# Lzcstan/DrugLAMP

Hardware: AMD Instinct MI355X
Metric: drug-protein pairs/sec training step (higher is better)
Workload: dtype bf16; 1 GPU; DrugLAMP training step (cls step, epoch 1; fwd+bwd+grad all-reduce+AdamW), BindingDB-shaped synthetic pairs (512 drug nodes/tokens, 2304 protein tokens = 256 sites, pre-extracted 384-d/640-d LLM embeddings), global batch 256 = 256 per GPU x 1; per_gpu_batch=256, global_batch=256, parallelism=dp1, step_kind=cls, epoch=1, hip_graph=False, protein_seq_len=2304, distinct_batches=8, first_touch_steps=8, padding_rows=computed once, protein_cnn_rows=distinct rows, streams=independent branches on side HIP streams

## Files before the change

### druglamp_amd/csrc/attention.hip

```cpp
#include "tiles.cuh"

namespace {
using namespace dltile;

struct AttnP {
  const char *Q, *K, *V, *O, *dO;
  char *Out, *dQ, *dK, *dV;
  float *LSE, *Delta, *raw;
  int64_t q_ps, q_hs, q_rs, k_ps, k_hs, k_rs, v_ps, v_hs, v_rs, o_ps, o_hs, o_rs, o_ss;
  int64_t do_ps, do_hs, do_rs, do_ss, dq_ps, dq_hs, dq_rs, dk_ps, dk_hs, dk_rs, dv_ps, dv_hs, dv_rs;
  int P, H, S, shift, Lq, Lk;
  float scale;
  int algo;
  int tail_start;
  float tail_bias;
};

template <int QT, int NKT>
__device__ __forceinline__ void add_tail_bias_t(f32x4 (&s)[QT][NKT], int k0, int g, int tail_start, float tb) {
#pragma unroll
  for (int kt = 0; kt < NKT; ++kt)
#pragma unroll
    for (int r = 0; r < 4; ++r)
      if (k0 + kt * 16 + 4 * g + r >= tail_start) {
// ... 334 lines not shown
  const T* d = reinterpret_cast<const T*>(p.dO) + (int64_t)seg * p.do_ss + (int64_t)pr * p.do_ps +
               (int64_t)h * p.do_hs + (int64_t)q * p.do_rs;
  float s = 0.f;
#pragma unroll
  for (int c = sub * 4; c < HD; c += 64) {
    const f32x4 a = load4<T>(o + c), b = load4<T>(d + c);
    s += a[0] * b[0] + a[1] * b[1] + a[2] * b[2] + a[3] * b[3];
  }
  s += __shfl_xor(s, 8, 64); s += __shfl_xor(s, 4, 64); s += __shfl_xor(s, 2, 64); s += __shfl_xor(s, 1, 64);
  if (sub == 0) p.Delta[row] = s;
}

template <typename T, int HD, int QT, bool RES>
__global__ __launch_bounds__(ATT_THREADS, (HD == 64 ? 2 : 1)) void attn_bwd_dq_kernel(const AttnP p) {
  using TL = ATile<T, HD>;
  constexpr int KF = Mma<T>::KF, NKF = HD / KF, NDT = HD / 16, CT = KF / 16;
  constexpr int KVB = 64, NKT = KVB / 16, NKP = KVB / KF;
  constexpr int QB = 4 * QT * 16;
  constexpr int LROWS = RES ? 256 : KVB;
  __shared__ __attribute__((aligned(16))) char smem[2 * LROWS * TL::RB];
  char* Ks = smem;
  char* Vs = smem + LROWS * TL::RB;
  const int lane = threadIdx.x & 63, wave = threadIdx.x >> 6, il = lane & 15, g = lane >> 4;
  const int qb = blockIdx.x, h = blockIdx.y, pq = blockIdx.z;
  const T* Qb = reinterpret_cast<const T*>(p.Q) + (int64_t)pq * p.q_ps + (int64_t)h * p.q_hs;
  const int qw0 = qb * QB + wave * QT * 16;
  const float c = p.scale * LOG2E;

  u32x4 qf[QT][NKF];
#pragma unroll
  for (int qt = 0; qt < QT; ++qt) {
    const int q = qw0 + qt * 16 + il;
#pragma unroll
    for (int kf = 0; kf < NKF; ++kf) qf[qt][kf] = frag_global<T>(Qb + (int64_t)q * p.q_rs, q < p.Lq, kf, g);
  }
  f32x4 dq[NDT][QT];
#pragma unroll
  for (int d = 0; d < NDT; ++d)
#pragma unroll
    for (int qt = 0; qt < QT; ++qt) dq[d][qt] = f32x4{0.f, 0.f, 0.f, 0.f};

  for (int seg = 0; seg < p.S; ++seg) {
    const int pa = seg == 0 ? pq : (pq + p.P - p.shift) % p.P;
    const T* Kb = reinterpret_cast<const T*>(p.K) + (int64_t)pa * p.k_ps + (int64_t)h * p.k_hs;
    const T* Vb = reinterpret_cast<const T*>(p.V) + (int64_t)pa * p.v_ps + (int64_t)h * p.v_hs;
    const T* dOb = reinterpret_cast<const T*>(p.dO) + (int64_t)seg * p.do_ss + (int64_t)pa * p.do_ps +
                   (int64_t)h * p.do_hs;
    const int64_t statbase = (((int64_t)seg * p.P + pa) * p.H + h) * p.Lq;
    const int nt = (p.Lk + KVB - 1) / KVB;
    if constexpr (RES) {
      dma_rows<T, HD, ATT_THREADS>(Ks, Kb, p.k_rs, p.Lk, nt * KVB);
      dma_rows<T, HD, ATT_THREADS>(Vs, Vb, p.v_rs, p.Lk, nt * KVB);
    }
    u32x4 dof[QT][NKF];
    float lse2[QT], delta[QT];
#pragma unroll
    for (int qt = 0; qt < QT; ++qt) {
      const int q = qw0 + qt * 16 + il;
      const bool ok = q < p.Lq;
#pragma unroll
      for (int kf = 0; kf < NKF; ++kf) dof[qt][kf] = frag_global<T>(dOb + (int64_t)q * p.do_rs, ok, kf, g);
      lse2[qt] = ok ? p.LSE[statbase + q] * LOG2E : INFINITY;
      if constexpr (sizeof(T) == 2) {
        const T* Ob = reinterpret_cast<const T*>(p.O) + (int64_t)seg * p.o_ss + (int64_t)pa * p.o_ps + (int64_t)h * p.o_hs;
        float part = 0.f;
#pragma unroll
        for (int kf = 0; kf < NKF; ++kf) part += dot8_bf16(dof[qt][kf], frag_global<T>(Ob + (int64_t)q * p.o_rs, ok, kf, g));
        delta[qt] = group4_sum(part);
        if (ok && g == 0) p.Delta[statbase + q] = delta[qt];
      } else {
        delta[qt] = ok ? p.Delta[statbase + q] : 0.f;
      }
    }
    Stager<T, HD, KVB> sk, sv;
    if constexpr (RES) {
      __syncthreads();
    } else {
      sk.load(Kb, p.k_rs, 0, p.Lk);
      sv.load(Vb, p.v_rs, 0, p.Lk);
    }
    for (int t = 0; t < nt; ++t) {
      const int k0 = t * KVB;
      if constexpr (!RES) {
        sk.store(Ks);
        sv.store(Vs);
        __syncthreads();
        if (t + 1 < nt) {
          sk.load(Kb, p.k_rs, k0 + KVB, p.Lk);
          sv.load(Vb, p.v_rs, k0 + KVB, p.Lk);
        }
      }
      const char* Kt = RES ? Ks + k0 * TL::RB : Ks;
      const char* Vt = RES ? Vs + k0 * TL::RB : Vs;
      f32x4 s[QT][NKT], dp[QT][NKT];
#pragma unroll
      for (int kt = 0; kt < NKT; ++kt) {
#pragma unroll
        for (int qt = 0; qt < QT; ++qt) { s[qt][kt] = f32x4{0.f, 0.f, 0.f, 0.f}; dp[qt][kt] = f32x4{0.f, 0.f, 0.f, 0.f}; }
#pragma unroll
        for (int kf = 0; kf < NKF; ++kf) {
          const u32x4 ka = frag_kc<T, HD>(Kt, kt * 16, kf, il, g);
          const u32x4 va = frag_kc<T, HD>(Vt, kt * 16, kf, il, g);
#pragma unroll
          for (int qt = 0; qt < QT; ++qt) {
            s[qt][kt] = Mma<T>::mma(ka, qf[qt][kf], s[qt][kt]);
            dp[qt][kt] = Mma<T>::mma(va, dof[qt][kf], dp[qt][kt]);
          }
        }
      }
      if constexpr (!RES) { if (k0 + KVB > p.tail_start) add_tail_bias_t<QT, NKT>(s, k0, g, p.tail_start, p.tail_bias); }
#pragma unroll
      for (int qt = 0; qt < QT; ++qt)
#pragma unroll
        for (int kt = 0; kt < NKT; ++kt)
#pragma unroll
          for (int r = 0; r < 4; ++r) {
            const float pv = fast_exp2(s[qt][kt][r] * c - lse2[qt]);
            s[qt][kt][r] = pv * (dp[qt][kt][r] - delta[qt]);
          }
#pragma unroll
      for (int kp = 0; kp < NKP; ++kp) {
        u32x4 db[QT];
#pragma unroll
        for (int qt = 0; qt < QT; ++qt) db[qt] = frag_from_acc<T>(&s[qt][kp * CT]);
#pragma unroll
        for (int d = 0; d < NDT; ++d) {
          const u32x4 kta = frag_tr<T, HD>(Kt, kp * KF, d * 16, il, g);
#pragma unroll
          for (int qt = 0; qt < QT; ++qt) dq[d][qt] = Mma<T>::mma(kta, db[qt], dq[d][qt]);
        }
      }
      if constexpr (!RES) __syncthreads();
    }
    if constexpr (RES) { if (seg + 1 < p.S) __syncthreads(); }
  }
  T* dQb = reinterpret_cast<T*>(p.dQ) + (int64_t)pq * p.dq_ps + (int64_t)h * p.dq_hs;
#pragma unroll
  for (int qt = 0; qt < QT; ++qt) {
    const int q = qw0 + qt * 16 + il;
    if (q < p.Lq) {
#pragma unroll
      for (int d = 0; d < NDT; ++d)
        store4_fam<4, T>(dQb + (int64_t)q * p.dq_rs + d * 16 + 4 * g, dq[d][qt] * p.scale);
    }
  }
}

__device__ __forceinline__ void att_dma16(const char* gsrc, uint32_t lds_off) {
  asm volatile("s_mov_b32 m0, %1\n\ts_nop 0\n\tglobal_load_lds_dwordx4 %0, off" ::"v"(gsrc), "s"(lds_off) : "memory");
}
__device__ __forceinline__ void att_wait_all() { asm volatile("s_waitcnt vmcnt(0) lgkmcnt(0)" ::: "memory"); }
__device__ __forceinline__ void att_barrier() { asm volatile("s_barrier" ::: "memory"); }

template <typename T, int HD, int QT, bool TAILK = false>
__global__ __launch_bounds__(ATT_THREADS, 2) void attn_bwd_dq_ring_kernel(const AttnP p) {
  using TL = ATile<T, HD>;
  constexpr int KF = Mma<T>::KF, NKF = HD / KF, NDT = HD / 16, CT = KF / 16;
  constexpr int KVB = 64, NKP = KVB / KF;
  constexpr int QB = 4 * QT * 16;
  constexpr int TILE = KVB * TL::RB, STAGE = 2 * TILE;
  constexpr int NCH = KVB * TL::CPR / ATT_THREADS;
  static_assert(sizeof(T) == 2 && KVB * TL::CPR % ATT_THREADS == 0, "bf16 tiles, whole DMA instructions");
  __shared__ __attribute__((aligned(16))) char smem[2 * STAGE];
  const uint32_t smem_lds = (uint32_t)(size_t)(__attribute__((address_space(3))) char*)smem;
  const int tid = threadIdx.x, lane = tid & 63, wave = tid >> 6, il = lane & 15, g = lane >> 4;
  const int qb = blockIdx.x, h = blockIdx.y, pq = blockIdx.z;
  const T* Qb = reinterpret_cast<const T*>(p.Q) + (int64_t)pq * p.q_ps + (int64_t)h * p.q_hs;
  const int qw0 = qb * QB + wave * QT * 16;
  const float c = p.scale * LOG2E;

  u32x4 qf[QT][NKF];
#pragma unroll
  for (int qt = 0; qt < QT; ++qt) {
    const int q = qw0 + qt * 16 + il;
#pragma unroll
    for (int kf = 0; kf < NKF; ++kf) qf[qt][kf] = frag_global<T>(Qb + (int64_t)q * p.q_rs, q < p.Lq, kf, g);
  }
  f32x4 dq[NDT][QT];
#pragma unroll
  for (int d = 0; d < NDT; ++d)
#pragma unroll
    for (int qt = 0; qt < QT; ++qt) dq[d][qt] = f32x4{0.f, 0.f, 0.f, 0.f};

  for (int seg = 0; seg < p.S; ++seg) {
    const int pa = seg == 0 ? pq : (pq + p.P - p.shift) % p.P;
    const T* Kb = reinterpret_cast<const T*>(p.K) + (int64_t)pa * p.k_ps + (int64_t)h * p.k_hs;
    const T* Vb = reinterpret_cast<const T*>(p.V) + (int64_t)pa * p.v_ps + (int64_t)h * p.v_hs;
    const T* dOb = reinterpret_cast<const T*>(p.dO) + (int64_t)seg * p.do_ss + (int64_t)pa * p.do_ps + (int64_t)h * p.do_hs;
    const int64_t statbase = (((int64_t)seg * p.P + pa) * p.H + h) * p.Lq;
    const int nt = (p.Lk + KVB - 1) / KVB;
    auto issue = [&](int t, int buf) {
      const char* zero = reinterpret_cast<const char*>(zero_page);
      const uint32_t sb = smem_lds + (uint32_t)buf * STAGE;
#pragma unroll
      for (int i = 0; i < NCH; ++i) {
        const int cc = tid + i * ATT_THREADS;
        const int row = cc / TL::CPR, ch = (cc % TL::CPR) ^ TL::swz(row);
        const int key = t * KVB + row;
        const char* ks = key < p.Lk ? reinterpret_cast<const char*>(Kb + (int64_t)key * p.k_rs + ch * TL::EPC) : zero;
        const char* vs = key < p.Lk ? reinterpret_cast<const char*>(Vb + (int64_t)key * p.v_rs + ch * TL::EPC) : zero;
        const uint32_t off = __builtin_amdgcn_readfirstlane((uint32_t)((wave * 64 + i * ATT_THREADS) * 16));
        att_dma16(ks, sb + off);
        att_dma16(vs, sb + TILE + off);
      }
    };
    if (seg > 0) att_barrier();
    issue(0, 0);
    u32x4 dof[QT][NKF];
    float lse2[QT], delta[QT];
#pragma unroll
    for (int qt = 0; qt < QT; ++qt) {
      const int q = qw0 + qt * 16 + il;
      const bool ok = q < p.Lq;
#pragma unroll
      for (int kf = 0; kf < NKF; ++kf) dof[qt][kf] = frag_global<T>(dOb + (int64_t)q * p.do_rs, ok, kf, g);
      lse2[qt] = ok ? p.LSE[statbase + q] * LOG2E : INFINITY;
      const T* Ob = reinterpret_cast<const T*>(p.O) + (int64_t)seg * p.o_ss + (int64_t)pa * p.o_ps + (int64_t)h * p.o_hs;
      float part = 0.f;
#pragma unroll
      for (int kf = 0; kf < NKF; ++kf) part += dot8_bf16(dof[qt][kf], frag_global<T>(Ob + (int64_t)q * p.o_rs, ok, kf, g));
      delta[qt] = group4_sum(part);
      if (ok && g == 0) p.Delta[statbase + q] = delta[qt];
    }
    for (int t = 0; t < nt; ++t) {
      att_wait_all();
      att_barrier();
      if (t + 1 < nt) issue(t + 1, (t + 1) & 1);
      const char* Kt = smem + (t & 1) * STAGE;
      const char* Vt = Kt + TILE;
#pragma unroll
      for (int kp = 0; kp < NKP; ++kp) {
        f32x4 s[QT][CT], dp[QT][CT];
#pragma unroll
        for (int ci = 0; ci < CT; ++ci) {
          const int kt = kp * CT + ci;
#pragma unroll
          for (int qt = 0; qt < QT; ++qt) { s[qt][ci] = f32x4{0.f, 0.f, 0.f, 0.f}; dp[qt][ci] = f32x4{0.f, 0.f, 0.f, 0.f}; }
#pragma unroll
          for (int kf = 0; kf < NKF; ++kf) {
            const u32x4 ka = frag_kc<T, HD>(Kt, kt * 16, kf, il, g);
            const u32x4 va = frag_kc<T, HD>(Vt, kt * 16, kf, il, g);
#pragma unroll
            for (int qt = 0; qt < QT; ++qt) {
              s[qt][ci] = Mma<T>::mma(ka, qf[qt][kf], s[qt][ci]);
              dp[qt][ci] = Mma<T>::mma(va, dof[qt][kf], dp[qt][ci]);
            }
          }
        }
        if constexpr (TAILK) {
          if (t * KVB + (kp + 1) * KF > p.tail_start) add_tail_bias_t<QT, CT>(s, t * KVB + kp * KF, g, p.tail_start, p.tail_bias);
        }
#pragma unroll
        for (int qt = 0; qt < QT; ++qt)
#pragma unroll
          for (int ci = 0; ci < CT; ++ci)
#pragma unroll
            for (int r = 0; r < 4; ++r) {
              const float pv = fast_exp2(s[qt][ci][r] * c - lse2[qt]);
              s[qt][ci][r] = pv * (dp[qt][ci][r] - delta[qt]);
            }
        u32x4 db[QT];
#pragma unroll
        for (int qt = 0; qt < QT; ++qt) db[qt] = frag_from_acc<T>(&s[qt][0]);
#pragma unroll
        for (int d = 0; d < NDT; ++d) {
          const u32x4 kta = frag_tr<T, HD>(Kt, kp * KF, d * 16, il, g);
#pragma unroll
          for (int qt = 0; qt < QT; ++qt) dq[d][qt] = Mma<T>::mma(kta, db[qt], dq[d][qt]);
        }
      }
    }
  }
  T* dQb = reinterpret_cast<T*>(p.dQ) + (int64_t)pq * p.dq_ps + (int64_t)h * p.dq_hs;
#pragma unroll
  for (int qt = 0; qt < QT; ++qt) {
    const int q = qw0 + qt * 16 + il;
    if (q < p.Lq) {
#pragma unroll
      for (int d = 0; d < NDT; ++d)
        store4_fam<4, T>(dQb + (int64_t)q * p.dq_rs + d * 16 + 4 * g, dq[d][qt] * p.scale);
    }
  }
}

template <typename T, int HD, int KT, bool RES>
__global__ __launch_bounds__(ATT_THREADS, (HD == 64 ? 2 : 1)) void attn_bwd_dkv_kernel(const AttnP p) {
  using TL = ATile<T, HD>;
  constexpr int KF = Mma<T>::KF, NKF = HD / KF, NDT = HD / 16, CT = KF / 16;
  constexpr int QSB = 64;
  constexpr int NQT = QSB / 16;
  constexpr int NQP = QSB / KF;
  constexpr int KVB = 4 * KT * 16;
  constexpr int LROWS = RES ? 256 : QSB;
  __shared__ __attribute__((aligned(16))) char smem[2 * LROWS * TL::RB + 2 * LROWS * sizeof(float)];
  char* Qs = smem;
  char* dOs = smem + LROWS * TL::RB;
  float* lse_s = reinterpret_cast<float*>(smem + 2 * LROWS * TL::RB);
  float* del_s = lse_s + LROWS;
  const int lane = threadIdx.x & 63, wave = threadIdx.x >> 6, il = lane & 15, g = lane >> 4;
  const int kb = blockIdx.x, h = blockIdx.y, pa = blockIdx.z;
  const T* Kb = reinterpret_cast<const T*>(p.K) + (int64_t)pa * p.k_ps + (int64_t)h * p.k_hs;
  const T* Vb = reinterpret_cast<const T*>(p.V) + (int64_t)pa * p.v_ps + (int64_t)h * p.v_hs;
  const int kw0 = kb * KVB + wave * KT * 16;
  const float c = p.scale * LOG2E;

  u32x4 kfr[KT][NKF], vfr[KT][NKF];
#pragma unroll
  for (int kt = 0; kt < KT; ++kt) {
    const int key = kw0 + kt * 16 + il;
    const bool ok = key < p.Lk;
#pragma unroll
    for (int kf = 0; kf < NKF; ++kf) {
      kfr[kt][kf] = frag_global<T>(Kb + (int64_t)key * p.k_rs, ok, kf, g);
      vfr[kt][kf] = frag_global<T>(Vb + (int64_t)key * p.v_rs, ok, kf, g);
    }
  }
  f32x4 dk[NDT][KT], dv[NDT][KT];
#pragma unroll
  for (int d = 0; d < NDT; ++d)
#pragma unroll
    for (int kt = 0; kt < KT; ++kt) { dk[d][kt] = f32x4{0.f, 0.f, 0.f, 0.f}; dv[d][kt] = f32x4{0.f, 0.f, 0.f, 0.f}; }
  const bool has_tail = !RES && kw0 + KT * 16 > p.tail_start;
  float kbl[KT];
#pragma unroll
  for (int kt = 0; kt < KT; ++kt) kbl[kt] = (kw0 + kt * 16 + il >= p.tail_start) ? p.tail_bias : 0.f;

  Stager<T, HD, QSB> sq, sdo;
  const int nqb = (p.Lq + QSB - 1) / QSB;
  for (int seg = 0; seg < p.S; ++seg) {
    const int qprob = seg == 0 ? pa : (pa + p.shift) % p.P;
    const T* Qb = reinterpret_cast<const T*>(p.Q) + (int64_t)qprob * p.q_ps + (int64_t)h * p.q_hs;
    const T* dOb = reinterpret_cast<const T*>(p.dO) + (int64_t)seg * p.do_ss + (int64_t)pa * p.do_ps +
                   (int64_t)h * p.do_hs;
    const int64_t statbase = (((int64_t)seg * p.P + pa) * p.H + h) * p.Lq;
    if constexpr (RES) {
      if (seg > 0) __syncthreads();
      dma_rows<T, HD, ATT_THREADS>(Qs, Qb, p.q_rs, p.Lq, nqb * QSB);
      dma_rows<T, HD, ATT_THREADS>(dOs, dOb, p.do_rs, p.Lq, nqb * QSB);
      for (int q = threadIdx.x; q < nqb * QSB; q += ATT_THREADS) {
        lse_s[q] = q < p.Lq ? p.LSE[statbase + q] * LOG2E : INFINITY;
        del_s[q] = q < p.Lq ? p.Delta[statbase + q] : 0.f;
      }
      __syncthreads();
    } else {
      sq.load(Qb, p.q_rs, 0, p.Lq);
      sdo.load(dOb, p.do_rs, 0, p.Lq);
    }
    for (int qb = 0; qb < nqb; ++qb) {
      const int q0 = qb * QSB;
      if constexpr (!RES) {
        sq.store(Qs);
        sdo.store(dOs);
        if (threadIdx.x < QSB) {
          const int q = q0 + threadIdx.x;
          lse_s[threadIdx.x] = q < p.Lq ? p.LSE[statbase + q] * LOG2E : INFINITY;
          del_s[threadIdx.x] = q < p.Lq ? p.Delta[statbase + q] : 0.f;
        }
        __syncthreads();
        if (qb + 1 < nqb) {
          sq.load(Qb, p.q_rs, q0 + QSB, p.Lq);
          sdo.load(dOb, p.do_rs, q0 + QSB, p.Lq);
        }
      }
      const char* Qt = RES ? Qs + q0 * TL::RB : Qs;
      const char* dOt = RES ? dOs + q0 * TL::RB : dOs;
      const float* lse_t = RES ? lse_s + q0 : lse_s;
      const float* del_t = RES ? del_s + q0 : del_s;
      f32x4 s[KT][NQT], dp[KT][NQT];
#pragma unroll
      for (int qt = 0; qt < NQT; ++qt) {
#pragma unroll
        for (int kt = 0; kt < KT; ++kt) { s[kt][qt] = f32x4{0.f, 0.f, 0.f, 0.f}; dp[kt][qt] = f32x4{0.f, 0.f, 0.f, 0.f}; }
#pragma unroll
        for (int kf = 0; kf < NKF; ++kf) {
          const u32x4 qa = frag_kc<T, HD>(Qt, qt * 16, kf, il, g);
          const u32x4 da = frag_kc<T, HD>(dOt, qt * 16, kf, il, g);
#pragma unroll
          for (int kt = 0; kt < KT; ++kt) {
            s[kt][qt] = Mma<T>::mma(qa, kfr[kt][kf], s[kt][qt]);
            dp[kt][qt] = Mma<T>::mma(da, vfr[kt][kf], dp[kt][qt]);
          }
        }
        const f32x4 l4 = *reinterpret_cast<const f32x4*>(lse_t + qt * 16 + 4 * g);
        const f32x4 d4 = *reinterpret_cast<const f32x4*>(del_t + qt * 16 + 4 * g);
        if (has_tail) {
#pragma unroll
          for (int kt = 0; kt < KT; ++kt) s[kt][qt] += kbl[kt];
        }
#pragma unroll
        for (int kt = 0; kt < KT; ++kt)
#pragma unroll
          for (int r = 0; r < 4; ++r) {
            const float pv = fast_exp2(s[kt][qt][r] * c - l4[r]);
            s[kt][qt][r] = pv;
            dp[kt][qt][r] = pv * (dp[kt][qt][r] - d4[r]);
          }
      }
#pragma unroll
      for (int qp = 0; qp < NQP; ++qp) {
        u32x4 pb[KT], sb[KT];
#pragma unroll
        for (int kt = 0; kt < KT; ++kt) {
          pb[kt] = frag_from_acc<T>(&s[kt][qp * CT]);
          sb[kt] = frag_from_acc<T>(&dp[kt][qp * CT]);
        }
#pragma unroll
        for (int d = 0; d < NDT; ++d) {
          const u32x4 dota = frag_tr<T, HD>(dOt, qp * KF, d * 16, il, g);
          const u32x4 qta = frag_tr<T, HD>(Qt, qp * KF, d * 16, il, g);
#pragma unroll
          for (int kt = 0; kt < KT; ++kt) {
            dv[d][kt] = Mma<T>::mma(dota, pb[kt], dv[d][kt]);
            dk[d][kt] = Mma<T>::mma(qta, sb[kt], dk[d][kt]);
          }
        }
      }
      if constexpr (!RES) __syncthreads();
    }
  }
  T* dKb = reinterpret_cast<T*>(p.dK) + (int64_t)pa * p.dk_ps + (int64_t)h * p.dk_hs;
  T* dVb = reinterpret_cast<T*>(p.dV) + (int64_t)pa * p.dv_ps + (int64_t)h * p.dv_hs;
#pragma unroll
  for (int kt = 0; kt < KT; ++kt) {
    const int key = kw0 + kt * 16 + il;
    if (key < p.Lk) {
#pragma unroll
      for (int d = 0; d < NDT; ++d) {
        store4_fam<4, T>(dKb + (int64_t)key * p.dk_rs + d * 16 + 4 * g, dk[d][kt] * p.scale);
        store4_fam<4, T>(dVb + (int64_t)key * p.dv_rs + d * 16 + 4 * g, dv[d][kt]);
      }
    }
  }
}

template <typename T, int HD, int KT, bool TAILK = false>
__global__ __launch_bounds__(ATT_THREADS, 1) void attn_bwd_dkv_ring_kernel(const AttnP p) {
  using TL = ATile<T, HD>;
  constexpr int KF = Mma<T>::KF, NKF = HD / KF, NDT = HD / 16, CT = KF / 16;
  constexpr int QSB = 64, NQP = QSB / KF;
  constexpr int KVB = 4 * KT * 16;
  constexpr int TILE = QSB * TL::RB, STAGE = 2 * TILE;
  constexpr int NCH = QSB * TL::CPR / ATT_THREADS;
  static_assert(sizeof(T) == 2 && QSB * TL::CPR % ATT_THREADS == 0, "bf16 tiles, whole DMA instructions");
  __shared__ __attribute__((aligned(16))) char smem[2 * STAGE + 2 * 2 * QSB * sizeof(float)];
  const uint32_t smem_lds = (uint32_t)(size_t)(__attribute__((address_space(3))) char*)smem;
  float* stat_s = reinterpret_cast<float*>(smem + 2 * STAGE);
  const int tid = threadIdx.x, lane = tid & 63, wave = tid >> 6, il = lane & 15, g = lane >> 4;
  const int kb = blockIdx.x, h = blockIdx.y, pa = blockIdx.z;
  const T* Kb = reinterpret_cast<const T*>(p.K) + (int64_t)pa * p.k_ps + (int64_t)h * p.k_hs;
  const T* Vb = reinterpret_cast<const T*>(p.V) + (int64_t)pa * p.v_ps + (int64_t)h * p.v_hs;
  const int kw0 = kb * KVB + wave * KT * 16;
  const float c = p.scale * LOG2E;

  u32x4 kfr[KT][NKF], vfr[KT][NKF];
#pragma unroll
  for (int kt = 0; kt < KT; ++kt) {
    const int key = kw0 + kt * 16 + il;
    const bool ok = key < p.Lk;
#pragma unroll
    for (int kf = 0; kf < NKF; ++kf) {
      kfr[kt][kf] = frag_global<T>(Kb + (int64_t)key * p.k_rs, ok, kf, g);
      vfr[kt][kf] = frag_global<T>(Vb + (int64_t)key * p.v_rs, ok, kf, g);
    }
  }
  f32x4 dk[NDT][KT], dv[NDT][KT];
#pragma unroll
  for (int d = 0; d < NDT; ++d)
#pragma unroll
    for (int kt = 0; kt < KT; ++kt) { dk[d][kt] = f32x4{0.f, 0.f, 0.f, 0.f}; dv[d][kt] = f32x4{0.f, 0.f, 0.f, 0.f}; }
  const bool has_tail = TAILK && kw0 + KT * 16 > p.tail_start;
  float kbl[KT];
#pragma unroll
  for (int kt = 0; kt < KT; ++kt) kbl[kt] = (TAILK && kw0 + kt * 16 + il >= p.tail_start) ? p.tail_bias : 0.f;

  const int nqb = (p.Lq + QSB - 1) / QSB;
  for (int seg = 0; seg < p.S; ++seg) {
    const int qprob = seg == 0 ? pa : (pa + p.shift) % p.P;
    const T* Qb = reinterpret_cast<const T*>(p.Q) + (int64_t)qprob * p.q_ps + (int64_t)h * p.q_hs;
    const T* dOb = reinterpret_cast<const T*>(p.dO) + (int64_t)seg * p.do_ss + (int64_t)pa * p.do_ps + (int64_t)h * p.do_hs;
    const int64_t statbase = (((int64_t)seg * p.P + pa) * p.H + h) * p.Lq;
    auto issue = [&](int qb, int buf) {
      const char* zero = reinterpret_cast<const char*>(zero_page);
      const uint32_t sb = smem_lds + (uint32_t)buf * STAGE;
#pragma unroll
      for (int i = 0; i < NCH; ++i) {
        const int cc = tid + i * ATT_THREADS;
        const int row = cc / TL::CPR, ch = (cc % TL::CPR) ^ TL::swz(row);
        const int q = qb * QSB + row;
        const char* qs_ = q < p.Lq ? reinterpret_cast<const char*>(Qb + (int64_t)q * p.q_rs + ch * TL::EPC) : zero;
        const char* ds_ = q < p.Lq ? reinterpret_cast<const char*>(dOb + (int64_t)q * p.do_rs + ch * TL::EPC) : zero;
        const uint32_t off = __builtin_amdgcn_readfirstlane((uint32_t)((wave * 64 + i * ATT_THREADS) * 16));
        att_dma16(qs_, sb + off);
        att_dma16(ds_, sb + TILE + off);
      }
      if (tid < QSB) {
        const int q = qb * QSB + tid;
        stat_s[(buf * 2 + 0) * QSB + tid] = q < p.Lq ? p.LSE[statbase + q] * LOG2E : INFINITY;
        stat_s[(buf * 2 + 1) * QSB + tid] = q < p.Lq ? p.Delta[statbase + q] : 0.f;
      }
    };
    if (seg > 0) att_barrier();
    issue(0, 0);
    for (int qb = 0; qb < nqb; ++qb) {
      att_wait_all();
      att_barrier();
      if (qb + 1 < nqb) issue(qb + 1, (qb + 1) & 1);
      const char* Qt = smem + (qb & 1) * STAGE;
      const char* dOt = Qt + TILE;
      const float* lse_t = stat_s + ((qb & 1) * 2 + 0) * QSB;
      const float* del_t = stat_s + ((qb & 1) * 2 + 1) * QSB;
#pragma unroll
      for (int qp = 0; qp < NQP; ++qp) {
        f32x4 s[KT][CT], dp[KT][CT];
#pragma unroll
        for (int ci = 0; ci < CT; ++ci) {
          const int qt = qp * CT + ci;
#pragma unroll
          for (int kt = 0; kt < KT; ++kt) { s[kt][ci] = f32x4{0.f, 0.f, 0.f, 0.f}; dp[kt][ci] = f32x4{0.f, 0.f, 0.f, 0.f}; }
#pragma unroll
          for (int kf = 0; kf < NKF; ++kf) {
            const u32x4 qa = frag_kc<T, HD>(Qt, qt * 16, kf, il, g);
            const u32x4 da = frag_kc<T, HD>(dOt, qt * 16, kf, il, g);
#pragma unroll
            for (int kt = 0; kt < KT; ++kt) {
              s[kt][ci] = Mma<T>::mma(qa, kfr[kt][kf], s[kt][ci]);
              dp[kt][ci] = Mma<T>::mma(da, vfr[kt][kf], dp[kt][ci]);
            }
          }
          const f32x4 l4 = *reinterpret_cast<const f32x4*>(lse_t + qt * 16 + 4 * g);
          const f32x4 d4 = *reinterpret_cast<const f32x4*>(del_t + qt * 16 + 4 * g);
          if (has_tail) {
#pragma unroll
            for (int kt = 0; kt < KT; ++kt) s[kt][ci] += kbl[kt];
          }
#pragma unroll
          for (int kt = 0; kt < KT; ++kt)
#pragma unroll
            for (int r = 0; r < 4; ++r) {
              const float pv = fast_exp2(s[kt][ci][r] * c - l4[r]);
              s[kt][ci][r] = pv;
              dp[kt][ci][r] = pv * (dp[kt][ci][r] - d4[r]);
            }
        }
        u32x4 pb[KT], sb[KT];
#pragma unroll
        for (int kt = 0; kt < KT; ++kt) {
          pb[kt] = frag_from_acc<T>(&s[kt][0]);
          sb[kt] = frag_from_acc<T>(&dp[kt][0]);
        }
#pragma unroll
        for (int d = 0; d < NDT; ++d) {
          const u32x4 dota = frag_tr<T, HD>(dOt, qp * KF, d * 16, il, g);
          const u32x4 qta = frag_tr<T, HD>(Qt, qp * KF, d * 16, il, g);
#pragma unroll
          for (int kt = 0; kt < KT; ++kt) {
            dv[d][kt] = Mma<T>::mma(dota, pb[kt], dv[d][kt]);
            dk[d][kt] = Mma<T>::mma(qta, sb[kt], dk[d][kt]);
          }
        }
      }
    }
  }
  T* dKb = reinterpret_cast<T*>(p.dK) + (int64_t)pa * p.dk_ps + (int64_t)h * p.dk_hs;
  T* dVb = reinterpret_cast<T*>(p.dV) + (int64_t)pa * p.dv_ps + (int64_t)h * p.dv_hs;
#pragma unroll
  for (int kt = 0; kt < KT; ++kt) {
    const int key = kw0 + kt * 16 + il;
    if (key < p.Lk) {
#pragma unroll
      for (int d = 0; d < NDT; ++d) {
        store4_fam<4, T>(dKb + (int64_t)key * p.dk_rs + d * 16 + 4 * g, dk[d][kt] * p.scale);
        store4_fam<4, T>(dVb + (int64_t)key * p.dv_rs + d * 16 + 4 * g, dv[d][kt]);
      }
    }
  }
}

__device__ __forceinline__ int ds_swz(int key) { return (((key >> 2) & 1) << 1) | ((key >> 3) & 1); }
template <typename T, int HD>
__global__ __launch_bounds__(512, 1) void attn_bwd_fused_kernel(const AttnP p) {
  static_assert(sizeof(T) == 2 && HD == 64, "bf16, head_dim 64");
  using TL = ATile<T, HD>;
  constexpr int KF = Mma<T>::KF, NKF = HD / KF, NDT = HD / 16, KT = 2, NQT = 2, QBLK = 32, NT = 512, NST = 4;
  constexpr int TILE = QBLK * TL::RB;
  constexpr int STAGE = 3 * TILE;
  constexpr int IMG = 256 * TL::RB;
  constexpr int DSB = 256 * 64;
  __shared__ __attribute__((aligned(16))) char smem[NST * STAGE + 2 * IMG + 2 * DSB + NST * (64 + QBLK) * (int)sizeof(float)];
  char* ring = smem;
  char* Ks = smem + NST * STAGE;
  char* Vs = Ks + IMG;
  char* dSs = Vs + IMG;
  float* lse_s = reinterpret_cast<float*>(dSs + 2 * DSB);
  float* del_s = lse_s + NST * 64;
  const int tid = threadIdx.x, lane = tid & 63, il = lane & 15, g = lane >> 4;
  const int wave = __builtin_amdgcn_readfirstlane(tid >> 6);
  const int h = blockIdx.y;
  const int a0 = blockIdx.z;
  const int npass = p.S == 2 ? 4 : 1;
  const int kw0 = wave * KT * 16;
  const int qt_o = wave & 1, dt_o = wave >> 1;
  const float c = p.scale * LOG2E;
  const int nblk = (p.Lq + QBLK - 1) / QBLK;
  const int G = npass * nblk;
  const uint32_t smem_base = (uint32_t)(size_t)(__attribute__((address_space(3))) char*)smem;
  const char* zero = reinterpret_cast<const char*>(zero_page);

  const int nd = wave <= 4 ? 2 : 1;
  int pf_pass = 0, pf_blk = 0, pf_stage = 0;
  const T* pfA = nullptr;
  const T* pfO = nullptr;
  const float* pfL = nullptr;
  int64_t pfA_rs = 0;
  auto pf_setup = [&]() {
    const int pa = pf_pass < 2 ? a0 : a0 + p.shift;
    const int seg = pf_pass & 1;
    const int qprob = seg == 0 ? pa : (pa + p.shift) % p.P;
    if (wave < 4) { pfA = reinterpret_cast<const T*>(p.Q) + ((int64_t)qprob * p.q_ps + (int64_t)h * p.q_hs); pfA_rs = p.q_rs; }
    else { pfA = reinterpret_cast<const T*>(p.dO) + ((int64_t)seg * p.do_ss + (int64_t)pa * p.do_ps + (int64_t)h * p.do_hs); pfA_rs = p.do_rs; }
    pfO = reinterpret_cast<const T*>(p.O) + ((int64_t)seg * p.o_ss + (int64_t)pa * p.o_ps + (int64_t)h * p.o_hs);
    pfL = p.LSE + (((int64_t)seg * p.P + pa) * p.H + h) * p.Lq;
  };
  pf_setup();
  auto issue_next = [&]() {
    const uint32_t st = smem_base + (uint32_t)(pf_stage * STAGE);
    const int row = 8 * (wave & 3) + (lane >> 3), q = pf_blk * QBLK + row;
    const int ch = (lane & 7) ^ TL::swz(row);
    const bool ok = q < p.Lq;
    lds_dma16(ok ? reinterpret_cast<const char*>(pfA + (int64_t)q * pfA_rs + ch * TL::EPC) : zero,
              st + (uint32_t)((wave < 4 ? 0 : TILE) + (wave & 3) * 1024));
    if (wave < 4) {
      lds_dma16(ok ? reinterpret_cast<const char*>(pfO + (int64_t)q * p.o_rs + ch * TL::EPC) : zero, st + (uint32_t)(2 * TILE + wave * 1024));
    } else if (wave == 4) {
      const int ql = pf_blk * QBLK + (lane & 31);
      lds_dma4(pfL + (ql < p.Lq ? ql : p.Lq - 1), smem_base + (uint32_t)((char*)lse_s - smem) + (uint32_t)(pf_stage * 256));
    }
    pf_stage = (pf_stage + 1) & (NST - 1);
    if (++pf_blk == nblk) {
      pf_blk = 0;
      if (++pf_pass < npass) pf_setup();
    }
  };
  auto issue_kv = [&](int pa) {
    const T* Kb = reinterpret_cast<const T*>(p.K) + (int64_t)pa * p.k_ps + (int64_t)h * p.k_hs;
    const T* Vb = reinterpret_cast<const T*>(p.V) + (int64_t)pa * p.v_ps + (int64_t)h * p.v_hs;
#pragma unroll
    for (int i = 0; i < 4; ++i) {
      const int row = (i * 8 + wave) * 8 + (lane >> 3);
      const int ch = (lane & 7) ^ TL::swz(row);
      const bool ok = row < p.Lk;
      lds_dma16(ok ? reinterpret_cast<const char*>(Kb + (int64_t)row * p.k_rs + ch * TL::EPC) : zero,
                smem_base + (uint32_t)(Ks - smem) + (uint32_t)((i * 8 + wave) * 1024));
      lds_dma16(ok ? reinterpret_cast<const char*>(Vb + (int64_t)row * p.v_rs + ch * TL::EPC) : zero,
                smem_base + (uint32_t)(Vs - smem) + (uint32_t)((i * 8 + wave) * 1024));
    }
  };
  auto form_delta = [&](int sg) {
    const char* st = ring + sg * STAGE;
    const int row = tid >> 4, off = TL::off(row, 4 * (tid & 15));
    const u32x2 a = *reinterpret_cast<const u32x2*>(st + TILE + off), b = *reinterpret_cast<const u32x2*>(st + 2 * TILE + off);
    float part = bf16lo(a[0]) * bf16lo(b[0]) + bf16hi(a[0]) * bf16hi(b[0]) + bf16lo(a[1]) * bf16lo(b[1]) + bf16hi(a[1]) * bf16hi(b[1]);
    part = row16_sum(part);
    if ((tid & 15) == 0) del_s[sg * QBLK + row] = part;
  };
  issue_kv(a0);
  for (int t = 0; t < 3 && t < G; ++t) issue_next();
  vm_wait<0>();
  __syncthreads();
  form_delta(0);
  if (G > 1) form_delta(1);
  __syncthreads();
  u32x4 kfr[KT][NKF], vfr[KT][NKF], ktr[8];
  f32x4 dk[NDT][KT], dv[NDT][KT];
  int gb = 0;
  for (int pass = 0; pass < npass; ++pass) {
    const int pa = pass < 2 ? a0 : a0 + p.shift;
    const int seg = pass & 1;
    const int qprob = seg == 0 ? pa : (pa + p.shift) % p.P;
    const bool new_kv = (pass & 1) == 0;
    if (new_kv) {
#pragma unroll
      for (int kt = 0; kt < KT; ++kt)
#pragma unroll
        for (int kf = 0; kf < NKF; ++kf) {
          kfr[kt][kf] = frag_kc<T, HD>(Ks, kw0 + kt * 16, kf, il, g);
          vfr[kt][kf] = frag_kc<T, HD>(Vs, kw0 + kt * 16, kf, il, g);
        }
#pragma unroll
      for (int cki = 0; cki < 8; ++cki) ktr[cki] = frag_tr<T, HD>(Ks, cki * 32, dt_o * 16, il, g);
#pragma unroll
      for (int d = 0; d < NDT; ++d)
#pragma unroll
        for (int kt = 0; kt < KT; ++kt) { dk[d][kt] = f32x4{0.f, 0.f, 0.f, 0.f}; dv[d][kt] = f32x4{0.f, 0.f, 0.f, 0.f}; }
    }
    T* dQb = reinterpret_cast<T*>(p.dQ) + (int64_t)qprob * p.dq_ps + (int64_t)h * p.dq_hs;
    const bool add_share = pass >= 2;
    for (int blk = 0; blk < nblk; ++blk, ++gb) {
      const int q0 = blk * QBLK;
      const int sg = gb & (NST - 1);
      const char* stg = ring + sg * STAGE;
      const char* Qt = stg;
      const char* dOt = stg + TILE;
      const float* lse_t = lse_s + sg * 64;
      const float* del_t = del_s + sg * QBLK;
      char* dSb = dSs + (gb & 1) * DSB;
      const int qo = q0 + qt_o * 16 + il;
      T* dst = dQb + (int64_t)(qo < p.Lq ? qo : p.Lq - 1) * p.dq_rs + dt_o * 16 + 4 * g;
      u32x2 prevw = {0u, 0u};
      if (add_share) asm volatile("global_load_dwordx2 %0, %1, off" : "=&v"(prevw) : "v"(dst) : "memory");
      const bool kv_now = npass == 4 && pass == 1 && blk == 0;
      if (kv_now) issue_kv(a0 + p.shift);
      if (gb + 3 < G) issue_next();
      u32x4 pb[KT], sb[KT];
#pragma unroll
// ... 9 lines not shown
          for (int kt = 0; kt < KT; ++kt) {
            s[kt] = Mma<T>::mma(qa, kfr[kt][kf], s[kt]);
            dp[kt] = Mma<T>::mma(da, vfr[kt][kf], dp[kt]);
          }
        }
        const f32x4 l4 = *reinterpret_cast<const f32x4*>(lse_t + qt * 16 + 4 * g) * LOG2E;
        const f32x4 d4 = *reinterpret_cast<const f32x4*>(del_t + qt * 16 + 4 * g);
#pragma unroll
        for (int kt = 0; kt < KT; ++kt) {
#pragma unroll
          for (int r = 0; r < 4; ++r) {
            const float pv = fast_exp2(s[kt][r] * c - l4[r]);
            s[kt][r] = pv;
            dp[kt][r] = pv * (dp[kt][r] - d4[r]);
          }
          pb[kt][2 * qt] = pack_bf16x2(s[kt][0], s[kt][1]);
          pb[kt][2 * qt + 1] = pack_bf16x2(s[kt][2], s[kt][3]);
          sb[kt][2 * qt] = pack_bf16x2(dp[kt][0], dp[kt][1]);
          sb[kt][2 * qt + 1] = pack_bf16x2(dp[kt][2], dp[kt][3]);
        }
      }
#pragma unroll
      for (int kt = 0; kt < KT; ++kt) {
        const int key = kw0 + kt * 16 + il, sw = ds_swz(key);
        *reinterpret_cast<u32x2*>(dSb + key * 64 + (((0 + (g >> 1)) ^ sw) << 4) + 8 * (g & 1)) = u32x2{sb[kt][0], sb[kt][1]};
        *reinterpret_cast<u32x2*>(dSb + key * 64 + (((2 + (g >> 1)) ^ sw) << 4) + 8 * (g & 1)) = u32x2{sb[kt][2], sb[kt][3]};
      }
#pragma unroll
      for (int d = 0; d < NDT; ++d) {
        const u32x4 dota = frag_tr<T, HD>(dOt, 0, d * 16, il, g);
        const u32x4 qta = frag_tr<T, HD>(Qt, 0, d * 16, il, g);
#pragma unroll
        for (int kt = 0; kt < KT; ++kt) {
          dv[d][kt] = Mma<T>::mma(dota, pb[kt], dv[d][kt]);
          dk[d][kt] = Mma<T>::mma(qta, sb[kt], dk[d][kt]);
        }
      }
      if (gb + 3 < G) {
        if (nd == 2) vm_wait<2>(); else vm_wait<1>();
      } else {
        vm_wait<0>();
      }
      __syncthreads();
      if (gb + 2 < G) form_delta((gb + 2) & (NST - 1));
      f32x4 dq = {0.f, 0.f, 0.f, 0.f};
#pragma unroll
      for (int cki = 0; cki < 8; ++cki) {
        const int r0 = cki * 32 + 4 * g + (il >> 2), sw = ds_swz(r0);
        const uint32_t off = (uint32_t)(r0 * 64 + (((2 * qt_o + ((il & 3) >> 1)) ^ sw) << 4) + (il & 1) * 8);
        const u32x2 lo = lds_read_tr16(dSb, off);
        const u32x2 hi = lds_read_tr16(dSb, off + 16 * 64);
        dq = Mma<T>::mma(ktr[cki], u32x4{lo[0], lo[1], hi[0], hi[1]}, dq);
      }
      if (add_share) asm volatile("s_waitcnt vmcnt(0)" : "+v"(prevw) :: "memory");
      if (qo < p.Lq) {
        f32x4 v = dq * p.scale;
        if (add_share) {
          v = v + f32x4{bf16lo(prevw[0]), bf16hi(prevw[0]), bf16lo(prevw[1]), bf16hi(prevw[1])};
          store4_fam<4, T>(dst, v);
        } else if (npass == 1) {
          store4_fam<4, T>(dst, v);
        } else {
          store4<T>(dst, v);
        }
      }
    }
    if (!new_kv || npass == 1) {
      T* dKb = reinterpret_cast<T*>(p.dK) + (int64_t)pa * p.dk_ps + (int64_t)h * p.dk_hs;
      T* dVb = reinterpret_cast<T*>(p.dV) + (int64_t)pa * p.dv_ps + (int64_t)h * p.dv_hs;
#pragma unroll
      for (int kt = 0; kt < KT; ++kt) {
        const int key = kw0 + kt * 16 + il;
        if (key < p.Lk) {
#pragma unroll
          for (int d = 0; d < NDT; ++d) {
            store4_fam<4, T>(dKb + (int64_t)key * p.dk_rs + d * 16 + 4 * g, dk[d][kt] * p.scale);
            store4_fam<4, T>(dVb + (int64_t)key * p.dv_rs + d * 16 + 4 * g, dv[d][kt]);
          }
        }
      }
    }
  }
}

template <typename T> constexpr int fwd_qt() { return sizeof(T) == 2 ? 2 : 1; }

int check_common(const char* who, int dtype, int head_dim, int nseg, int P, int H, int Lq, int Lk,
                 const int64_t* strides, int nstrides) {
  DL_CHECK_ARG(dtype == DL_F32 || dtype == DL_BF16, DL_ERR_ARG, "%s: bad dtype", who);
  DL_CHECK_ARG(head_dim == 64 || head_dim == 128, DL_ERR_UNSUPPORTED, "%s: head_dim %d not in {64,128}", who, head_dim);
  DL_CHECK_ARG(nseg == 1 || nseg == 2, DL_ERR_ARG, "%s: n_segments must be 1 or 2", who);
  DL_CHECK_ARG(P > 0 && H > 0 && Lq > 0 && Lk > 0 && P <= 65535 && H <= 65535, DL_ERR_SHAPE, "%s: bad sizes", who);
  const int epc = 16 / (int)dl_dtype_size(dtype);
  for (int i = 0; i < nstrides; ++i)
    DL_CHECK_ARG(strides[i] % epc == 0, DL_ERR_ALIGN, "%s: stride #%d (%ld) not a multiple of %d elements", who,
                 i, (long)strides[i], epc);
  return DL_OK;
}

template <typename T, int HD>
int launch_fwd(const AttnP& p, hipStream_t s) {
  if constexpr (sizeof(T) == 2) {
    if (HD == 64 && p.Lk <= 256 && p.algo != DL_ATTN_ALGO_STREAM && p.tail_start >= p.Lk) {
      constexpr int NW = HD == 64 ? 4 : 8;
      hipLaunchKernelGGL((attn_fwd_res_kernel<T, HD, 2, NW>), dim3((uint32_t)p.H, (uint32_t)p.P), dim3(64 * NW), 0, s, p);
      return DL_OK;
    }
  }
  constexpr int QT = fwd_qt<T>();
  constexpr int QB = 4 * QT * 16;
  dim3 grid((uint32_t)(p.S * ((p.Lq + QB - 1) / QB)), (uint32_t)p.H, (uint32_t)p.P);
  if constexpr (sizeof(T) == 2 && HD == 64) {
    if (!p.raw && p.Lq <= 64) {
      const dim3 g1((uint32_t)(p.S * ((p.Lq + 63) / 64)), (uint32_t)p.H, (uint32_t)p.P);
      hipLaunchKernelGGL((attn_fwd_kernel<T, HD, 1, 64, 4>), g1, dim3(ATT_THREADS), 0, s, p);
      return DL_OK;
    }
    if (!p.raw && p.Lk >= 1024) {
      hipLaunchKernelGGL((attn_fwd_kernel<T, HD, QT, 128>), grid, dim3(ATT_THREADS), 0, s, p);
      return DL_OK;
    }
  }
  hipLaunchKernelGGL((attn_fwd_kernel<T, HD, QT>), grid, dim3(ATT_THREADS), 0, s, p);
  return DL_OK;
}

template <typename T, int HD>
int launch_bwd(const AttnP& p, hipStream_t s) {
  constexpr int QT = fwd_qt<T>();
  constexpr int QB = 4 * QT * 16;
  constexpr int KT = sizeof(T) == 2 ? 2 : 1;
  constexpr int KVB = 4 * KT * 16;
  const dim3 gq((uint32_t)((p.Lq + QB - 1) / QB), (uint32_t)p.H, (uint32_t)p.P);
  const dim3 gk((uint32_t)((p.Lk + KVB - 1) / KVB), (uint32_t)p.H, (uint32_t)p.P);
  if constexpr (sizeof(T) == 2 && HD == 64) {
    const int64_t nwg = (int64_t)p.H * (p.S == 2 ? p.shift : p.P);
    if (p.Lk <= 256 && (p.S == 1 || 2 * p.shift == p.P) && p.tail_start >= p.Lk &&
        (p.algo == DL_ATTN_ALGO_ONE_PASS || (p.algo == DL_ATTN_ALGO_AUTO && nwg >= 256))) {
      const dim3 gf(1u, (uint32_t)p.H, (uint32_t)(p.S == 2 ? p.shift : p.P));
      hipLaunchKernelGGL((attn_bwd_fused_kernel<T, HD>), gf, dim3(512), 0, s, p);
      return DL_OK;
    }
    if (p.Lk <= 256 && p.Lq <= 256 && p.algo != DL_ATTN_ALGO_STREAM && p.tail_start >= p.Lk) {
      hipLaunchKernelGGL((attn_bwd_dq_kernel<T, HD, QT, true>), gq, dim3(ATT_THREADS), 0, s, p);
      hipLaunchKernelGGL((attn_bwd_dkv_kernel<T, HD, KT, true>), gk, dim3(ATT_THREADS), 0, s, p);
      return DL_OK;
    }
  }
  if constexpr (sizeof(T) != 2) {
    const int64_t rows = (int64_t)p.S * p.P * p.H * p.Lq;
    hipLaunchKernelGGL((attn_delta_kernel<T, HD>), dim3((uint32_t)((rows + 15) / 16)), dim3(256), 0, s, p);
  }
  if constexpr (sizeof(T) == 2 && HD == 128) {
    if (p.tail_start < p.Lk) {
      hipLaunchKernelGGL((attn_bwd_dq_ring_kernel<T, HD, QT, true>), gq, dim3(ATT_THREADS), 0, s, p);
      hipLaunchKernelGGL((attn_bwd_dkv_ring_kernel<T, HD, KT, true>), gk, dim3(ATT_THREADS), 0, s, p);
    } else {
      hipLaunchKernelGGL((attn_bwd_dq_ring_kernel<T, HD, QT>), gq, dim3(ATT_THREADS), 0, s, p);
      hipLaunchKernelGGL((attn_bwd_dkv_ring_kernel<T, HD, KT>), gk, dim3(ATT_THREADS), 0, s, p);
    }
  } else {
    hipLaunchKernelGGL((attn_bwd_dq_kernel<T, HD, QT, false>), gq, dim3(ATT_THREADS), 0, s, p);
    hipLaunchKernelGGL((attn_bwd_dkv_kernel<T, HD, KT, false>), gk, dim3(ATT_THREADS), 0, s, p);
  }
  return DL_OK;
}

template <typename Args>
int fill_common(const char* who, const Args* a, AttnP& p) {
  p.Q = (const char*)a->Q; p.K = (const char*)a->K; p.V = (const char*)a->V;
  p.q_ps = a->q_ps; p.q_hs = a->q_hs; p.q_rs = a->q_rs; p.k_ps = a->k_ps; p.k_hs = a->k_hs; p.k_rs = a->k_rs;
  p.v_ps = a->v_ps; p.v_hs = a->v_hs; p.v_rs = a->v_rs; p.o_ps = a->o_ps; p.o_hs = a->o_hs; p.o_rs = a->o_rs;
  p.o_ss = a->o_ss;
  p.P = a->n_problems; p.H = a->n_heads; p.S = a->n_segments; p.shift = a->partner_shift;
  p.Lq = a->Lq; p.Lk = a->Lk; p.scale = a->scale; p.algo = a->algo;
  DL_CHECK_ARG(a->key_tail_rows >= 0 && a->key_tail_rows <= a->Lk && (a->key_tail_rows == 0 || (a->key_tail_weight >= 1.f && a->scale > 0.f)),
               DL_ERR_ARG, "%s: key_tail_rows in [0, Lk], key_tail_weight >= 1", who);
  DL_CHECK_ARG(a->key_tail_rows == 0 || a->n_segments == 1, DL_ERR_UNSUPPORTED, "%s: key multiplicities with one segment only", who);
  p.tail_start = a->Lk - a->key_tail_rows;
  p.tail_bias = a->key_tail_rows ? logf(a->key_tail_weight) / a->scale : 0.f;
  return DL_OK;
}

}

extern "C" int dl_attn_fwd(const dl_attn_fwd_args* a, dl_stream stream) {
  hipStream_t s = (hipStream_t)stream;
  DL_CHECK_ARG(a && a->Q && a->K && a->V && a->O, DL_ERR_ARG, "dl_attn_fwd: null pointer");
  const int64_t st[] = {a->q_ps, a->q_hs, a->q_rs, a->k_ps, a->k_hs, a->k_rs, a->v_ps, a->v_hs,
                        a->v_rs, a->o_ps, a->o_hs, a->o_rs, a->o_ss};
  int rc = check_common("dl_attn_fwd", a->dtype, a->head_dim, a->n_segments, a->n_problems, a->n_heads,
                        a->Lq, a->Lk, st, 13);
  if (rc != DL_OK) return rc;
  DL_CHECK_ARG(a->n_segments == 1 || (a->partner_shift >= 0 && a->partner_shift < a->n_problems),
               DL_ERR_ARG, "dl_attn_fwd: bad partner_shift");
  AttnP p = {};
  rc = fill_common("dl_attn_fwd", a, p);
  if (rc != DL_OK) return rc;
  p.Out = (char*)a->O; p.LSE = a->LSE; p.raw = a->raw_logits;
  dl_prof_before(1, s);
  if (a->dtype == DL_BF16) rc = a->head_dim == 64 ? launch_fwd<bf16_t, 64>(p, s) : launch_fwd<bf16_t, 128>(p, s);
  else rc = a->head_dim == 64 ? launch_fwd<float, 64>(p, s) : launch_fwd<float, 128>(p, s);
  DL_CHECK_LAUNCH("dl_attn_fwd");
  const double nq = (double)a->n_segments * a->n_problems * a->n_heads * a->Lq;
  const int es = (int)dl_dtype_size(a->dtype);
  dl_prof_after(1, s, 4.0 * nq * a->Lk * a->head_dim,
                (2.0 * nq + 2.0 * a->n_problems * a->n_heads * a->Lk) * a->head_dim * es);
  return rc;
}

extern "C" int dl_attn_bwd(const dl_attn_bwd_args* a, dl_stream stream) {
  hipStream_t s = (hipStream_t)stream;
  DL_CHECK_ARG(a && a->Q && a->K && a->V && a->O && a->dO && a->LSE && a->Delta && a->dQ && a->dK && a->dV,
               DL_ERR_ARG, "dl_attn_bwd: null pointer");
  const int64_t st[] = {a->q_ps, a->q_hs, a->q_rs, a->k_ps, a->k_hs, a->k_rs, a->v_ps, a->v_hs, a->v_rs,
                        a->o_ps, a->o_hs, a->o_rs, a->o_ss, a->do_ps, a->do_hs, a->do_rs, a->do_ss,
                        a->dq_ps, a->dq_hs, a->dq_rs, a->dk_ps, a->dk_hs, a->dk_rs, a->dv_ps, a->dv_hs, a->dv_rs};
  int rc = check_common("dl_attn_bwd", a->dtype, a->head_dim, a->n_segments, a->n_problems, a->n_heads,
                        a->Lq, a->Lk, st, 26);
  if (rc != DL_OK) return rc;
  DL_CHECK_ARG(a->n_segments == 1 || (a->partner_shift >= 0 && a->partner_shift < a->n_problems),
               DL_ERR_ARG, "dl_attn_bwd: bad partner_shift");
  AttnP p = {};
  rc = fill_common("dl_attn_bwd", a, p);
  if (rc != DL_OK) return rc;
  p.O = (const char*)a->O; p.dO = (const char*)a->dO; p.LSE = const_cast<float*>(a->LSE); p.Delta = a->Delta;
  p.dQ = (char*)a->dQ; p.dK = (char*)a->dK; p.dV = (char*)a->dV;
  p.do_ps = a->do_ps; p.do_hs = a->do_hs; p.do_rs = a->do_rs; p.do_ss = a->do_ss;
  p.dq_ps = a->dq_ps; p.dq_hs = a->dq_hs; p.dq_rs = a->dq_rs; p.dk_ps = a->dk_ps; p.dk_hs = a->dk_hs;
  p.dk_rs = a->dk_rs; p.dv_ps = a->dv_ps; p.dv_hs = a->dv_hs; p.dv_rs = a->dv_rs;
  dl_prof_before(2, s);
  if (a->dtype == DL_BF16) rc = a->head_dim == 64 ? launch_bwd<bf16_t, 64>(p, s) : launch_bwd<bf16_t, 128>(p, s);
  else rc = a->head_dim == 64 ? launch_bwd<float, 64>(p, s) : launch_bwd<float, 128>(p, s);
  DL_CHECK_LAUNCH("dl_attn_bwd");
  const double nq = (double)a->n_segments * a->n_problems * a->n_heads * a->Lq;
  const int es = (int)dl_dtype_size(a->dtype);
  dl_prof_after(2, s, 10.0 * nq * a->Lk * a->head_dim,
                (4.0 * nq + 4.0 * a->n_problems * a->n_heads * a->Lk) * a->head_dim * es);
  return rc;
}
```

Baseline: 20890 pairs/s.

## Retune dK/dV ring backward for occupancy and cheaper DMA address math

The dK/dV ring backward kernel now uses one key tile per wave (RKT=1) and declares occupancy 2 in launch bounds, giving a larger grid and more resident workgroups. Both ring kernels hoist the per-thread row/chunk/swizzle offsets out of the DMA issue loop, so each piece only adds a scalar row base. The LSE/Delta stat loads are held in registers and written to LDS one iteration later, so their global latency overlaps the tile wait. A small asm barrier pins the K/V fragments after the wait. Fewer key rows per wave means Q/dO tiles are reloaded more often, which trades data reuse for parallelism.

Result: no change. 21080 pairs/s (median of 6 runs) (+0.9%).

```diff
diff --git a/druglamp_amd/csrc/attention.hip b/druglamp_amd/csrc/attention.hip
--- a/druglamp_amd/csrc/attention.hip
+++ b/druglamp_amd/csrc/attention.hip
@@ -510,6 +510,14 @@
 __device__ __forceinline__ void att_wait_all() { asm volatile("s_waitcnt vmcnt(0) lgkmcnt(0)" ::: "memory"); }
 __device__ __forceinline__ void att_barrier() { asm volatile("s_barrier" ::: "memory"); }
 
+template <int A, int B>
+__device__ __forceinline__ void att_landed(u32x4 (&x)[A][B], u32x4 (&y)[A][B]) {
+#pragma unroll
+  for (int a = 0; a < A; ++a)
+#pragma unroll
+    for (int b = 0; b < B; ++b) asm volatile("" : "+v"(x[a][b]), "+v"(y[a][b]));
+}
+
 template <typename T, int HD, int QT, bool TAILK = false>
 __global__ __launch_bounds__(ATT_THREADS, 2) void attn_bwd_dq_ring_kernel(const AttnP p) {
   using TL = ATile<T, HD>;
@@ -526,6 +534,10 @@
   const T* Qb = reinterpret_cast<const T*>(p.Q) + (int64_t)pq * p.q_ps + (int64_t)h * p.q_hs;
   const int qw0 = qb * QB + wave * QT * 16;
   const float c = p.scale * LOG2E;
+  constexpr int RPI = ATT_THREADS / TL::CPR;
+  static_assert(ATT_THREADS % TL::CPR == 0 && RPI % 8 == 0, "a thread keeps its chunk and its swizzle from piece to piece");
+  const int row0 = tid / TL::CPR, ch0 = (tid % TL::CPR) ^ TL::swz(row0);
+  const int64_t koff = (int64_t)row0 * p.k_rs + ch0 * TL::EPC, voff = (int64_t)row0 * p.v_rs + ch0 * TL::EPC;
 
   u32x4 qf[QT][NKF];
 #pragma unroll
@@ -548,15 +560,15 @@
     const int64_t statbase = (((int64_t)seg * p.P + pa) * p.H + h) * p.Lq;
     const int nt = (p.Lk + KVB - 1) / KVB;
     auto issue = [&](int t, int buf) {
+      asm volatile("" : "+s"(t));
       const char* zero = reinterpret_cast<const char*>(zero_page);
       const uint32_t sb = smem_lds + (uint32_t)buf * STAGE;
 #pragma unroll
       for (int i = 0; i < NCH; ++i) {
-        const int cc = tid + i * ATT_THREADS;
-        const int row = cc / TL::CPR, ch = (cc % TL::CPR) ^ TL::swz(row);
-        const int key = t * KVB + row;
-        const char* ks = key < p.Lk ? reinterpret_cast<const char*>(Kb + (int64_t)key * p.k_rs + ch * TL::EPC) : zero;
-        const char* vs = key < p.Lk ? reinterpret_cast<const char*>(Vb + (int64_t)key * p.v_rs + ch * TL::EPC) : zero;
+        const int kr = t * KVB + i * RPI;
+        const bool ok = kr + row0 < p.Lk;
+        const char* ks = ok ? reinterpret_cast<const char*>(Kb + (int64_t)kr * p.k_rs + koff) : zero;
+        const char* vs = ok ? reinterpret_cast<const char*>(Vb + (int64_t)kr * p.v_rs + voff) : zero;
         const uint32_t off = __builtin_amdgcn_readfirstlane((uint32_t)((wave * 64 + i * ATT_THREADS) * 16));
         att_dma16(ks, sb + off);
         att_dma16(vs, sb + TILE + off);
@@ -792,7 +804,7 @@
 }
 
 template <typename T, int HD, int KT, bool TAILK = false>
-__global__ __launch_bounds__(ATT_THREADS, 1) void attn_bwd_dkv_ring_kernel(const AttnP p) {
+__global__ __launch_bounds__(ATT_THREADS, 2) void attn_bwd_dkv_ring_kernel(const AttnP p) {
   using TL = ATile<T, HD>;
   constexpr int KF = Mma<T>::KF, NKF = HD / KF, NDT = HD / 16, CT = KF / 16;
   constexpr int QSB = 64, NQP = QSB / KF;
@@ -809,6 +821,10 @@
   const T* Vb = reinterpret_cast<const T*>(p.V) + (int64_t)pa * p.v_ps + (int64_t)h * p.v_hs;
   const int kw0 = kb * KVB + wave * KT * 16;
   const float c = p.scale * LOG2E;
+  constexpr int RPI = ATT_THREADS / TL::CPR;
+  static_assert(ATT_THREADS % TL::CPR == 0 && RPI % 8 == 0, "a thread keeps its chunk and its swizzle from piece to piece");
+  const int row0 = tid / TL::CPR, ch0 = (tid % TL::CPR) ^ TL::swz(row0);
+  const int64_t qoff = (int64_t)row0 * p.q_rs + ch0 * TL::EPC, dooff = (int64_t)row0 * p.do_rs + ch0 * TL::EPC;
 
   u32x4 kfr[KT][NKF], vfr[KT][NKF];
 #pragma unroll
@@ -832,35 +848,44 @@
   for (int kt = 0; kt < KT; ++kt) kbl[kt] = (TAILK && kw0 + kt * 16 + il >= p.tail_start) ? p.tail_bias : 0.f;
 
   const int nqb = (p.Lq + QSB - 1) / QSB;
+  float lse_n = INFINITY, del_n = 0.f;
   for (int seg = 0; seg < p.S; ++seg) {
     const int qprob = seg == 0 ? pa : (pa + p.shift) % p.P;
     const T* Qb = reinterpret_cast<const T*>(p.Q) + (int64_t)qprob * p.q_ps + (int64_t)h * p.q_hs;
     const T* dOb = reinterpret_cast<const T*>(p.dO) + (int64_t)seg * p.do_ss + (int64_t)pa * p.do_ps + (int64_t)h * p.do_hs;
     const int64_t statbase = (((int64_t)seg * p.P + pa) * p.H + h) * p.Lq;
     auto issue = [&](int qb, int buf) {
+      asm volatile("" : "+s"(qb));
       const char* zero = reinterpret_cast<const char*>(zero_page);
       const uint32_t sb = smem_lds + (uint32_t)buf * STAGE;
 #pragma unroll
       for (int i = 0; i < NCH; ++i) {
-        const int cc = tid + i * ATT_THREADS;
-        const int row = cc / TL::CPR, ch = (cc % TL::CPR) ^ TL::swz(row);
-        const int q = qb * QSB + row;
-        const char* qs_ = q < p.Lq ? reinterpret_cast<const char*>(Qb + (int64_t)q * p.q_rs + ch * TL::EPC) : zero;
-        const char* ds_ = q < p.Lq ? reinterpret_cast<const char*>(dOb + (int64_t)q * p.do_rs + ch * TL::EPC) : zero;
+        const int qr = qb * QSB + i * RPI;
+        const bool ok = qr + row0 < p.Lq;
+        const char* qs_ = ok ? reinterpret_cast<const char*>(Qb + (int64_t)qr * p.q_rs + qoff) : zero;
+        const char* ds_ = ok ? reinterpret_cast<const char*>(dOb + (int64_t)qr * p.do_rs + dooff) : zero;
         const uint32_t off = __builtin_amdgcn_readfirstlane((uint32_t)((wave * 64 + i * ATT_THREADS) * 16));
         att_dma16(qs_, sb + off);
         att_dma16(ds_, sb + TILE + off);
       }
       if (tid < QSB) {
         const int q = qb * QSB + tid;
-        stat_s[(buf * 2 + 0) * QSB + tid] = q < p.Lq ? p.LSE[statbase + q] * LOG2E : INFINITY;
-        stat_s[(buf * 2 + 1) * QSB + tid] = q < p.Lq ? p.Delta[statbase + q] : 0.f;
+        lse_n = q < p.Lq ? p.LSE[statbase + q] : INFINITY;
+        del_n = q < p.Lq ? p.Delta[statbase + q] : 0.f;
+      }
+    };
+    auto put_stat = [&](int buf) {
+      if (tid < QSB) {
+        stat_s[(buf * 2 + 0) * QSB + tid] = lse_n * LOG2E;
+        stat_s[(buf * 2 + 1) * QSB + tid] = del_n;
       }
     };
     if (seg > 0) att_barrier();
     issue(0, 0);
     for (int qb = 0; qb < nqb; ++qb) {
+      put_stat(qb & 1);
       att_wait_all();
+      att_landed(kfr, vfr);
       att_barrier();
       if (qb + 1 < nqb) issue(qb + 1, (qb + 1) & 1);
       const char* Qt = smem + (qb & 1) * STAGE;
@@ -918,6 +943,7 @@
         }
       }
     }
+    asm volatile("" ::"v"(lse_n), "v"(del_n));
   }
   T* dKb = reinterpret_cast<T*>(p.dK) + (int64_t)pa * p.dk_ps + (int64_t)h * p.dk_hs;
   T* dVb = reinterpret_cast<T*>(p.dV) + (int64_t)pa * p.dv_ps + (int64_t)h * p.dv_hs;
@@ -1233,12 +1259,14 @@
     hipLaunchKernelGGL((attn_delta_kernel<T, HD>), dim3((uint32_t)((rows + 15) / 16)), dim3(256), 0, s, p);
   }
   if constexpr (sizeof(T) == 2 && HD == 128) {
+    constexpr int RKT = 1;
+    const dim3 gr((uint32_t)((p.Lk + 4 * RKT * 16 - 1) / (4 * RKT * 16)), (uint32_t)p.H, (uint32_t)p.P);
     if (p.tail_start < p.Lk) {
       hipLaunchKernelGGL((attn_bwd_dq_ring_kernel<T, HD, QT, true>), gq, dim3(ATT_THREADS), 0, s, p);
-      hipLaunchKernelGGL((attn_bwd_dkv_ring_kernel<T, HD, KT, true>), gk, dim3(ATT_THREADS), 0, s, p);
+      hipLaunchKernelGGL((attn_bwd_dkv_ring_kernel<T, HD, RKT, true>), gr, dim3(ATT_THREADS), 0, s, p);
     } else {
       hipLaunchKernelGGL((attn_bwd_dq_ring_kernel<T, HD, QT>), gq, dim3(ATT_THREADS), 0, s, p);
-      hipLaunchKernelGGL((attn_bwd_dkv_ring_kernel<T, HD, KT>), gk, dim3(ATT_THREADS), 0, s, p);
+      hipLaunchKernelGGL((attn_bwd_dkv_ring_kernel<T, HD, RKT>), gr, dim3(ATT_THREADS), 0, s, p);
     }
   } else {
     hipLaunchKernelGGL((attn_bwd_dq_kernel<T, HD, QT, false>), gq, dim3(ATT_THREADS), 0, s, p);
```
